# keio-bioinformatics/stem_kernel

Measured on AMD Instinct MI355X. Metric: sequence-pairs/sec (Gram entries/s) at L=200 nt, higher is better.
Workload: dtype f64

## Files before the change

stem_kernel_amd/csrc/kernels/dag_stem.hip:

```cpp
#include <hip/hip_runtime.h>

#include <algorithm>

#include "device_set.h"
#include "launch.h"

namespace sk {

__global__ void sk_prep_kernel(DevSet s, DevParamNodes pn, const double* __restrict__ gpow,
                               double gap2) {
  const int e = blockIdx.x * blockDim.x + threadIdx.x;
  if (e >= s.n_examples) return;
  const int nl = s.ex_nl[e];
  const int nb = s.ex_node_base[e], eb = s.ex_edge_base[e];
  for (int k = 0; k < nl; ++k) {
    const uint32_t a = s.nd_a[nb + k];
    const int e0 = a & 0xffff, ne = (a >> 16) & 0xff;
    const double v_s = gap2 * (double)s.nd_w[nb + k];
    double L = 0.0, SL = 0.0;
    if (ne == 0) {
      L += 1.0 * v_s * gpow[s.nd_c[nb + k]];
    } else {
      for (int t = 0; t < ne; ++t) {
        const uint32_t ed = s.ed[eb + e0 + t].x;
        const double gp = gpow[ed >> 16];
        const double Lc = pn.nd_L[nb + (ed & 0xffff)];
        L += Lc * v_s * gp;
        SL += gp * Lc;
      }
    }
    pn.nd_L[nb + k] = L;
    pn.nd_SL[nb + k] = SL;
  }
  for (int r = 0; r < nl; ++r) pn.xr_SL[nb + r] = pn.nd_SL[nb + s.xr_node[nb + r]];
  {
    int k = s.ex_xch_base[e];
    for (int r = 0; r < nl; ++r) {
      const int ne = s.xrow[nb + r].a & 0xff;
      for (int t = 0; t < ne; ++t, ++k) pn.xr_chw[k] = gpow[s.xr_ch[k] >> 16];
    }
  }
  if (s.n_gam > 0) {
    const int gb = s.ex_xg_base[e], nlg = s.ex_nlxg[e];
    int k = s.ex_xgch_base[e];
    int pk = s.n_phi > 0 ? s.ex_phk_base[e] : 0;
    for (int r = 0; r < nlg; ++r) {
      const double SLr = pn.nd_SL[nb + s.xg_node[gb + r]];
      pn.xg_SL[gb + r] = SLr;
      const XRow xr = s.xgrow[gb + r];
      const int ne = xr.a & 0xff;
      for (int t = 0; t < ne; ++t, ++k) {
        const uint32_t c = s.xg_ch[k];
        const double wc = gpow[c >> 16] * gpow[s.xg_clg[k]] * (double)s.xg_cpf[k];
        double w;
        switch (s.xg_cty[k]) {
          case 0: w = gpow[c >> 16]; break;
          case 1: w = wc; break;
          case 2: w = (double)xr.bp0 * wc; break;
          case 3: w = (double)xr.bp0 * SLr; break;
          default: w = gap2 * (double)xr.w * wc; break;
        }
        pn.xg_chw[k] = w;
        if (s.xg_cty[k] == 2) pn.phk_w[pk++] = xr.P * w;
      }
    }
    double* h = pn.gam_h + (int64_t)e * s.n_gam;
    for (int g = 0; g < s.n_gam; ++g) h[g] = 0.0;
    for (int i = s.ex_gr_base[e]; i < s.ex_gr_base[e + 1]; ++i) {
      const uint32_t inf = s.gr_info[i];
      h[inf & 0xffff] += s.gr_P[i] * (gpow[inf >> 16] * (double)s.gr_pf[i]);
    }
    if (s.n_phi > 0)
      for (int i = s.ex_gra_base[e]; i < s.ex_gra_base[e + 1]; ++i) {
        const uint32_t r = s.gra_row[i];
        h[s.gra_gidx[i]] += s.xgrow[r].P * ((double)s.xgrow[r].bp0 * pn.xg_SL[r]);
      }
  }
}

typedef __attribute__((address_space(3))) double lds_f64;
typedef __attribute__((address_space(3))) float lds_f32;
typedef __attribute__((address_space(3))) uint32_t lds_u32;
typedef __attribute__((address_space(3))) int32_t lds_i32;

struct YView {
  const uint4* __restrict__ nrg;
  const lds_u32* sc;
  const lds_f64* ew;
  const lds_f32* ewf;
  const lds_f64* gp;
  double gap2;
  const lds_u32* ed2;
  const uint32_t* __restrict__ ed2g;
  const lds_i32* lfirst;
  const lds_i32* ycs;
  int lmax;
  int nl, nch;
  float nseqs;
  int nb, bb;
};

#if defined(__HIP_DEVICE_COMPILE__)
template <typename T>
using cst_ptr = const __attribute__((address_space(4))) T*;
#else
template <typename T>
using cst_ptr = const T*;
#endif

__device__ __forceinline__ void wave_sync() {
  __builtin_amdgcn_fence(__ATOMIC_RELEASE, "wavefront");
  __builtin_amdgcn_wave_barrier();
  __builtin_amdgcn_fence(__ATOMIC_ACQUIRE, "wavefront");
}

#define SCHED_FENCE() __builtin_amdgcn_sched_barrier(0)
#ifndef SK_W20
#define SK_W20 8
#endif
#ifndef SK_W16
#define SK_W16 8
#endif
#ifndef SK_NPF12
#define SK_NPF12 2
#endif
#ifndef SK_NPF20
#define SK_NPF20 2
#endif
#ifndef SK_NPF16
#define SK_NPF16 1
#endif
#ifndef SK_NPF17
#define SK_NPF17 0
#endif
#ifndef SK_PW
#define SK_PW 3
#endif
#ifndef SK_SEGSUM
#define SK_SEGSUM 1
#endif
#ifndef SK_SEGSUM_MAXK
#define SK_SEGSUM_MAXK 20
#endif
#ifndef SK_MU
#define SK_MU 3
#endif
#ifndef SK_NODEW_MIN
#define SK_NODEW_MIN 20
#endif
#ifndef SK_M16
#define SK_M16 1
#endif
#ifndef SK_K17
#define SK_K17 1
#endif
template <int MAXK>
constexpr bool m16_wide() {
  return (MAXK == 16 || MAXK == 17) && SK_M16 != 0;
}
template <int MAXK>
constexpr bool node_weights() {
  return MAXK >= SK_NODEW_MIN || m16_wide<MAXK>();
}
#ifndef SK_NODEF_MIN
#define SK_NODEF_MIN 24
#endif
template <int MAXK>
constexpr bool node_weights_f32() {
  return node_weights<MAXK>() && MAXK >= SK_NODEF_MIN;
}
#ifndef SK_PW2_MIN
#define SK_PW2_MIN 24
#endif
template <int MAXK>
#ifndef SK_PW17
#define SK_PW17 2
#endif
constexpr int pass_width() {
  return MAXK == 17 ? SK_PW17 : (MAXK >= SK_PW2_MIN || m16_wide<MAXK>()) ? 2 : SK_PW;
}
static inline bool m16_wide_of(int maxk) { return (maxk == 16 || maxk == 17) && SK_M16 != 0; }
static inline int pass_width_of(int maxk) {
  return maxk == 17 ? SK_PW17 : (maxk >= SK_PW2_MIN || m16_wide_of(maxk)) ? 2 : SK_PW;
}
static inline bool node_weights_of(int maxk) { return maxk >= SK_NODEW_MIN || m16_wide_of(maxk); }
#ifndef SK_EDG_MIN
#define SK_EDG_MIN 64
#endif
template <int MAXK>
constexpr bool edges_global() {
  return MAXK >= SK_EDG_MIN;
}

#ifdef SK_STAMPS
#define STAMP(i)                                                  \
  do {                                                            \
    __builtin_amdgcn_sched_barrier(0);                            \
    const unsigned long long _t = __builtin_amdgcn_s_memtime();   \
    tacc[i] += _t - tlast;                                        \
    tlast = _t;                                                   \
    __builtin_amdgcn_sched_barrier(0);                            \
  } while (0)
#else
#define STAMP(i) do {} while (0)
#endif

__device__ __forceinline__ double match_node_score(const lds_f64* co, const DevSet& s, int xbb,
                                                int xb0, int xnb, const DevSet& ys, const YView& Y,
                                                int yb0, int ynb, double xwg, double ywg,
                                                double x_nbp, double y_nbp, double x_nseq) {
  double v = 0.0;
  for (int a = 0; a < xnb; ++a) {
    const double cx = (double)s.bpf_p[xbb + xb0 + a];
    const uint32_t ca = s.bpf_code[xbb + xb0 + a] * 16u;
    for (int b = 0; b < ynb; ++b) {
      const double cy = (double)ys.bpf_p[Y.bb + yb0 + b];
      v += co[ca + ys.bpf_code[Y.bb + yb0 + b]] * cx * cy;
    }
  }
  v += ywg * x_nbp / x_nseq;
  v += xwg * y_nbp / (double)Y.nseqs;
  return v;
}

__device__ __forceinline__ __amdgpu_buffer_rsrc_t row_rsrc(const double* base, int nly) {
  const uint64_t a = (uint64_t)base;
  const uint32_t lo = __builtin_amdgcn_readfirstlane((uint32_t)a);
  const uint32_t hi = __builtin_amdgcn_readfirstlane((uint32_t)(a >> 32));
  return __builtin_amdgcn_make_buffer_rsrc((void*)(((uint64_t)hi << 32) | lo), (short)0,
                                           __builtin_amdgcn_readfirstlane(nly * 8), 0x00020000);
}

#ifndef SK_ROW_LD_POL
#define SK_ROW_LD_POL 0
#endif
#ifndef SK_ROW_ST_POL
#define SK_ROW_ST_POL 0
#endif
typedef unsigned int u32x2 __attribute__((__vector_size__(2 * sizeof(unsigned int))));

__device__ __forceinline__ double row_ld(__amdgpu_buffer_rsrc_t r, int lane, int k) {
  return __builtin_bit_cast(double, __builtin_amdgcn_raw_buffer_load_b64(r, lane * 8, k * 512, SK_ROW_LD_POL));
}

#ifndef SK_HALF_A
#define SK_HALF_A 64
#endif
#ifndef SK_HALF_D
#define SK_HALF_D 64
#endif
#ifndef SK_M16_HALFA
#define SK_M16_HALFA 1
#endif
#ifndef SK_M16_HALFD
#define SK_M16_HALFD 1
#endif
template <int MAXK>
__device__ __forceinline__ void add_rows2(double (&S)[MAXK], __amdgpu_buffer_rsrc_t r0,
                                          __amdgpu_buffer_rsrc_t r1, double eg0, double eg1,
                                          int lane) {
  constexpr int H = (MAXK > SK_HALF_A || (m16_wide<MAXK>() && SK_M16_HALFA)) ? (MAXK + 1) / 2 : MAXK;
#pragma unroll
  for (int h0 = 0; h0 < MAXK; h0 += H) {
    double a[H], b[H];
#pragma unroll
    for (int k = 0; k < H; ++k) {
      a[k] = h0 + k < MAXK ? row_ld(r0, lane, h0 + k) : 0.0;
      b[k] = h0 + k < MAXK ? row_ld(r1, lane, h0 + k) : 0.0;
    }
    SCHED_FENCE();
#pragma unroll
    for (int k = 0; k < H; ++k)
      if (h0 + k < MAXK) S[h0 + k] += eg0 * a[k] + eg1 * b[k];
  }
}

template <bool NW, bool NWF>
__device__ __forceinline__ void iy_sweep(const YView& Y, lds_f64* R, int c0, int lane) {
  const lds_u32* rp = Y.sc + c0 * 64 + lane;
  const lds_f64* wp = Y.ew + (NW ? 0 : c0 * 64 + lane);
  auto nweight = [&](uint32_t rec) __attribute__((always_inline)) -> double {
    const uint32_t pa = (rec >> 11) & 0x7ff;
    return (NWF ? Y.gap2 * (double)Y.ewf[pa] : Y.ew[pa]) * Y.gp[rec >> 22];
  };
  struct Ck {
    uint32_t rec;
    double w, rv;
  };
  Ck A, B, C;
  A.rec = rp[0];
  B.rec = rp[64];
  A.w = NW ? nweight(A.rec) : wp[0];
  B.w = 0.0;
  C.rec = 0u;
  C.w = C.rv = B.rv = 0.0;
  A.rv = R[A.rec & 0x7ff];
  int c = c0;
  const int nch = Y.nch;
  auto step = [&](Ck& X, Ck& Yc, Ck& Z) __attribute__((always_inline)) -> bool {
    Z.rec = rp[128];
    Yc.w = NW ? nweight(Yc.rec) : wp[64];
    __hip_atomic_fetch_add(&R[(X.rec >> 11) & 0x7ff], X.rv * X.w, __ATOMIC_RELAXED,
                           __HIP_MEMORY_SCOPE_WAVEFRONT);
    Yc.rv = R[Yc.rec & 0x7ff];
    rp += 64;
    wp += 64;
    return ++c < nch;
  };
  for (;;) {
    if (!step(A, B, C)) break;
    if (!step(B, C, A)) break;
    if (!step(C, A, B)) break;
  }
  wave_sync();
}

__device__ __forceinline__ const double* child_row(uint32_t c, const double* slab, const double* gamtab,
                                                   const double* phitab, int stride) {
  const double* base = (c & 0x8000u) ? gamtab : (c & 0x4000u) ? phitab : slab;
  return base + (size_t)(c & 0x3fffu) * stride;
}

template <int MAXK>
__device__ double stem_pair(const StemLaunch& P, const YView& Y, lds_f64* R, lds_f64* hb,
                            const lds_f64* co, const lds_f64* gp, double* __restrict__ slab, int x,
                            int lane, bool gam, const double* __restrict__ gamtab,
                            const lds_f64* kap, const double* __restrict__ phitab,
                            const double* __restrict__ phikap) {
  constexpr int stride = 64 * MAXK;
  constexpr int PW = pass_width<MAXK>();
  const DevSet& s = P.xset;
  const DevSet& ys = P.yset;
  const double* __restrict__ yPg = ys.yn_P + Y.nb;
  const int NLy = Y.nl;
  if (s.ex_nl[x] == 0 || NLy == 0) return 0.0;
  const int xnb = s.ex_node_base[x], xbb = s.ex_bpf_base[x];
  const int xgb = gam ? s.ex_xg_base[x] : 0;
  const int nlx = gam ? s.ex_nlxg[x] : s.ex_nl[x];
  int chp = gam ? s.ex_xgch_base[x] : s.ex_xch_base[x];
  const double x_nseq = (double)s.ex_nseqs[x];
  const double gap2 = P.gap2;
  const int band = (int)P.band;
  const XRow* __restrict__ xrows = gam ? s.xgrow + xgb : s.xrow + xnb;
  const double* __restrict__ xsl = gam ? P.pn.xg_SL + xgb : P.pn.xr_SL + xnb;
  const uint32_t* __restrict__ xch = gam ? s.xg_ch : s.xr_ch;
  const double* __restrict__ xchw = gam ? P.pn.xg_chw : P.pn.xr_chw;
  double kacc = 0.0;
  if (gam) {
    const double* __restrict__ h = P.pn.gam_h + (int64_t)x * s.n_gam;
    for (int g = lane; g < s.n_gam; g += 64) kacc += h[g] * kap[g];
    if (P.phi_on)
      for (int j = s.ex_phk_base[x] + lane; j < s.ex_phk_base[x + 1]; j += 64)
        kacc += P.pn.phk_w[j] * phikap[s.phk_idx[j]];
  }
  if (nlx == 0) {
    for (int off = 32; off > 0; off >>= 1) kacc += __shfl_xor(kacc, off, 64);
    return kacc;
  }
#ifdef SK_STAMPS
  unsigned long long tacc[8] = {0, 0, 0, 0, 0, 0, 0, 0};
  unsigned long long cnt[4] = {0, 0, 0, 0};
  unsigned long long tlast = __builtin_amdgcn_s_memtime();
#endif

  const cst_ptr<XRow> xrows_c = (cst_ptr<XRow>)xrows;
  const cst_ptr<double> xsl_c = (cst_ptr<double>)xsl;
  const cst_ptr<uint32_t> xch_c = (cst_ptr<uint32_t>)xch;
  const cst_ptr<double> xchw_c = (cst_ptr<double>)xchw;
  XRow nx = xrows_c[0];
  double nSL = xsl_c[0];
  uint32_t nch[4];
  double ncw[4];
#pragma unroll
  for (int j = 0; j < 4; ++j) {
    nch[j] = xch_c[chp + j];
    ncw[j] = xchw_c[chp + j];
  }

  double S[MAXK];
#pragma unroll
  for (int k = 0; k < MAXK; ++k) S[k] = 0.0;
  uint32_t done = 0;

  for (int r = 0; r < nlx; ++r) {
    const uint32_t xa = nx.a, xb = nx.b, xc = nx.c;
    const double xwg = gap2 * (double)nx.w;
    const double x_nbp = (double)nx.nbp;
    const double xP = nx.P, xSL = nSL, xpf = (double)nx.bp0;
    uint32_t ch[4];
    double cw[4];
#pragma unroll
    for (int j = 0; j < 4; ++j) {
      ch[j] = nch[j];
      cw[j] = ncw[j];
    }
    const int xne = xa & 0xff, xnbf = (xa >> 8) & 0xff;
    const int chp_r = chp;
    chp += xne;
    const int xlen = xb & 0xffff;
    const uint32_t pslot = xb >> 16;
    const int xb0 = xc & 0xffff;
    const bool xloop = xne == 0;
    const double xeg0 = gp[xa >> 16];
    const bool x_one = xnbf == 1 && x_nbp == 0.0;
    const uint32_t xcode = ((xc >> 16) & 0xffu) * 16u;
    const bool combo = (xc >> 31) != 0u;
    int qa = 0, qb = NLy;
    if (band > 0) {
      qa = Y.lfirst[min(max(xlen - band, 0), Y.lmax + 1)];
      qb = Y.lfirst[min(max(xlen + band + 1, 0), Y.lmax + 1)];
    }
    qa = __builtin_amdgcn_readfirstlane(qa);
    qb = __builtin_amdgcn_readfirstlane(qb);
    uint4 nd_first[PW];
    double Pq_first[PW];
#pragma unroll
    for (int j = 0; j < PW; ++j) {
      nd_first[j] = make_uint4(0u, 0u, 0u, 0u);
      Pq_first[j] = 0.0;
    }
    if (qa < qb) {
#pragma unroll
      for (int j = 0; j < PW; ++j) {
        const int qf = min(max(qb - 64 * PW, qa) + 64 * j + lane, qb - 1);
        nd_first[j] = Y.nrg[qf];
        Pq_first[j] = yPg[qf];
      }
    }
    STAMP(0);

    SCHED_FENCE();
    if (r + 1 < nlx) {
      nx = xrows_c[r + 1];
      nSL = xsl_c[r + 1];
#pragma unroll
      for (int j = 0; j < 4; ++j) {
        nch[j] = xch_c[chp + j];
        ncw[j] = xchw_c[chp + j];
      }
    }
    SCHED_FENCE();

    {
      uint32_t c[4] = {0u, 0u, 0u, 0u};
      double w[4] = {0.0, 0.0, 0.0, 0.0};
      int na = 0;
#pragma unroll
      for (int j = 0; j < 4; ++j) {
        const bool take = j < xne && !(done >> j & 1u);
        c[0] = (take && na == 0) ? ch[j] : c[0];
        c[1] = (take && na == 1) ? ch[j] : c[1];
        c[2] = (take && na == 2) ? ch[j] : c[2];
        c[3] = (take && na == 3) ? ch[j] : c[3];
        w[0] = (take && na == 0) ? cw[j] : w[0];
        w[1] = (take && na == 1) ? cw[j] : w[1];
        w[2] = (take && na == 2) ? cw[j] : w[2];
        w[3] = (take && na == 3) ? cw[j] : w[3];
        na += take ? 1 : 0;
      }
      for (int h = 0; h < 4; h += 2) {
        if (na > h) {
          const bool two = na > h + 1;
          const uint32_t c0 = c[h], c1 = two ? c[h + 1] : c[h];
          const double eg0 = w[h], eg1 = two ? w[h + 1] : 0.0;
          add_rows2<MAXK>(S, row_rsrc(child_row(c0, slab, gamtab, phitab, stride), NLy),
                          row_rsrc(child_row(c1, slab, gamtab, phitab, stride), NLy), eg0, eg1, lane);
        }
      }
    }
#ifdef SK_STAMPS
    {
      int nl_ = 0;
      for (int j = 0; j < 4; ++j) nl_ += (j < xne && !(done >> j & 1u)) ? 1 : 0;
      cnt[0] += nl_ + (xne > 4 ? xne - 4 : 0);
    }
#endif
    for (int t = 4; t < xne; t += 2) {
      const uint32_t c0 = xch[chp_r + t];
      const bool two = t + 1 < xne;
      const uint32_t c1 = two ? xch[chp_r + t + 1] : c0;
      const double eg0 = xchw[chp_r + t], eg1 = two ? xchw[chp_r + t + 1] : 0.0;
      add_rows2<MAXK>(S, row_rsrc(child_row(c0, slab, gamtab, phitab, stride), NLy),
                      row_rsrc(child_row(c1, slab, gamtab, phitab, stride), NLy), eg0, eg1, lane);
    }
    STAMP(1);

    if (!combo) {
#pragma unroll
      for (int k = 0; k < MAXK; ++k) R[lane + 64 * k] = lane + 64 * k < qb ? S[k] : 0.0;
    }
    double rowk = 0.0;
    STAMP(2);
#ifdef SK_STAMPS
    cnt[3] += qb > qa ? qb - qa : 0;
#endif
    if (!combo && qa < qb) {
      constexpr int NW = 64 * PW;
      int top = qb - 1, q0 = max(top - NW + 1, qa);
      uint4 nd_n[PW];
      double Pq_n[PW];
#pragma unroll
      for (int j = 0; j < PW; ++j) {
        nd_n[j] = nd_first[j];
        Pq_n[j] = Pq_first[j];
      }
      for (;;) {
        uint4 nd[PW];
        double Pq[PW];
#pragma unroll
        for (int j = 0; j < PW; ++j) {
          nd[j] = nd_n[j];
          Pq[j] = Pq_n[j];
        }
        const int ntop = top - NW, nq0 = max(ntop - NW + 1, qa);
        if (ntop >= qa) {
#pragma unroll
          for (int j = 0; j < PW; ++j) {
            nd_n[j] = Y.nrg[min(nq0 + 64 * j + lane, ntop)];
            Pq_n[j] = yPg[min(nq0 + 64 * j + lane, ntop)];
          }
        }
        double co_v[PW], gl_v[PW];
#pragma unroll
        for (int j = 0; j < PW; ++j) {
          co_v[j] = co[xcode + ((nd[j].y >> 16) & 0xf)];
          gl_v[j] = gp[nd[j].y & 0xffff];
        }
        double Hq[PW];
#pragma unroll
        for (int j = 0; j < PW; ++j) Hq[j] = 0.0;
        if (!xloop) {
          const int ea = __builtin_amdgcn_readfirstlane(nd[0].x & 0xffff);
          const int jt = (top - q0) >> 6;
          uint32_t ndt = nd[0].x;
#pragma unroll
          for (int j = 1; j < PW; ++j) ndt = jt == j ? nd[j].x : ndt;
          const uint32_t at = __builtin_amdgcn_readlane(ndt, (top - q0) & 63);
          const int eb = (int)((at & 0xffff) + ((at >> 16) & 0xff));
          constexpr bool EG = edges_global<MAXK>();
          uint32_t en[SK_MU];
          if constexpr (EG) {
#pragma unroll
            for (int u = 0; u < SK_MU; ++u) en[u] = Y.ed2g[min(ea + 64 * u + lane, eb - 1)];
          }
          for (int f0 = ea; f0 < eb; f0 += 64 * SK_MU) {
            uint32_t e[SK_MU];
            if constexpr (EG) {
#pragma unroll
              for (int u = 0; u < SK_MU; ++u) {
                e[u] = en[u];
                en[u] = Y.ed2g[min(f0 + 64 * (SK_MU + u) + lane, eb - 1)];
              }
            } else {
#pragma unroll
              for (int u = 0; u < SK_MU; ++u) e[u] = Y.ed2[min(f0 + 64 * u + lane, eb - 1)];
            }
            double g[SK_MU], rv[SK_MU];
#pragma unroll
            for (int u = 0; u < SK_MU; ++u) {
              g[u] = gp[e[u] >> 22];
              rv[u] = R[e[u] & 0x7ff];
            }
#pragma unroll
            for (int u = 0; u < SK_MU; ++u) {
              const bool ok = f0 + 64 * u + lane < eb;
              const double w = g[u] * rv[u] * (ok ? 1.0 : 0.0);
              const int h = ok ? (int)((e[u] >> 11) & 0x7ff) - q0 : lane;
              if constexpr (SK_SEGSUM && MAXK <= SK_SEGSUM_MAXK) {
                const int key = ok ? h : -1 - lane;
                const int ql = lane & 3;
                double sw = w;
                {
                  const int ks = __builtin_amdgcn_mov_dpp(key, 0x90, 0xf, 0xf, false);
                  const double ws = __hiloint2double(
                      __builtin_amdgcn_mov_dpp(__double2hiint(sw), 0x90, 0xf, 0xf, false),
                      __builtin_amdgcn_mov_dpp(__double2loint(sw), 0x90, 0xf, 0xf, false));
                  sw += (ql >= 1 && ks == key) ? ws : 0.0;
                }
                {
                  const int ks = __builtin_amdgcn_mov_dpp(key, 0x40, 0xf, 0xf, false);
                  const double ws = __hiloint2double(
                      __builtin_amdgcn_mov_dpp(__double2hiint(sw), 0x40, 0xf, 0xf, false),
                      __builtin_amdgcn_mov_dpp(__double2loint(sw), 0x40, 0xf, 0xf, false));
                  sw += (ql >= 2 && ks == key) ? ws : 0.0;
                }
                const int kn = __builtin_amdgcn_mov_dpp(key, 0xF9, 0xf, 0xf, false);
                if (ok && (ql == 3 || kn != key))
                  __hip_atomic_fetch_add(&hb[h], sw, __ATOMIC_RELAXED, __HIP_MEMORY_SCOPE_WAVEFRONT);
              } else {
                __hip_atomic_fetch_add(&hb[h], w, __ATOMIC_RELAXED, __HIP_MEMORY_SCOPE_WAVEFRONT);
              }
            }
          }
#pragma unroll
          for (int j = 0; j < PW; ++j) {
            Hq[j] = hb[64 * j + lane];
            hb[64 * j + lane] = 0.0;
          }
        }
#pragma unroll
        for (int j = 0; j < PW; ++j) {
          const int q = q0 + 64 * j + lane;
          const bool on = q <= top;
          const uint32_t nda = nd[j].x, ndc = nd[j].y;
          double H = Hq[j];
          if (((nda >> 16) & 0xff) == 0)
            H = (xloop ? xeg0 : xSL) * gl_v[j];
          double vs;
          if (x_one && (ndc >> 24) != 0u) {
            vs = co_v[j] * xpf * (double)__uint_as_float(nd[j].w);
          } else {
            const int qq = on ? q : top;
            vs = H != 0.0 ? match_node_score(co, s, xbb, xb0, xnbf, ys, Y, ys.yn_b[Y.nb + qq] >> 16,
                                             nda >> 24, xwg, gap2 * (double)__uint_as_float(nd[j].z),
                                             x_nbp, (double)ys.yn_nbp[Y.nb + qq], x_nseq)
                          : 0.0;
          }
          const double M = vs * H;
          if (on) {
            R[q] = M;
            rowk += M * Pq[j];
          }
        }
#ifdef SK_STAMPS
        cnt[2] += 1;
#endif
        if (ntop < qa) break;
        top = ntop;
        q0 = nq0;
      }
    }
    STAMP(3);
#pragma unroll
    for (int k = 0; k < MAXK; ++k) {
      const int q = lane + 64 * k;
      if (!combo && 64 * k < qa && q < qa) R[q] = 0.0;
    }
    kacc += xP * rowk;
    wave_sync();
    STAMP(4);

    constexpr int NPF = MAXK == 17 ? SK_NPF17
                        : (MAXK == 16 && (SK_NPF16 == 0 || SK_M16 == 2)) ? 0
                        : ((MAXK <= 12 && SK_NPF12 == 2) || (MAXK == 16 && SK_NPF16 == 2) ||
                           (MAXK == 20 && SK_W20 == 8 && SK_NPF20 == 2)) ? 2 : 1;
    uint32_t nxt_done = 0;
    double egd = 0.0, egt0 = 0.0, egt1 = 0.0;
    double T0[MAXK], T1[MAXK];
#pragma unroll
    for (int k = 0; k < MAXK; ++k) T0[k] = T1[k] = 0.0;
    if (r + 1 < nlx) {
      const int nne = nx.a & 0xff;
      uint32_t pf0 = 0, pf1 = 0;
      int npf = 0;
#pragma unroll
      for (int j = 0; j < 4; ++j) {
        if (j < nne) {
          const uint32_t c = nch[j];
          const double g = ncw[j];
          if ((c & 0xffff) == pslot) {
            egd += g;
            nxt_done |= 1u << j;
          } else if (npf < NPF) {
            if (npf == 0) {
              pf0 = c;
              egt0 = g;
            } else {
              pf1 = c;
              egt1 = g;
            }
            ++npf;
            nxt_done |= 1u << j;
          }
        }
      }
      if (NPF >= 1 && npf >= 1) {
        const __amdgpu_buffer_rsrc_t r0 = row_rsrc(child_row(pf0, slab, gamtab, phitab, stride), NLy);
#pragma unroll
        for (int k = 0; k < MAXK; ++k) T0[k] = row_ld(r0, lane, k);
      }
      if (NPF >= 2 && npf >= 2) {
        const __amdgpu_buffer_rsrc_t r1 = row_rsrc(child_row(pf1, slab, gamtab, phitab, stride), NLy);
#pragma unroll
        for (int k = 0; k < MAXK; ++k) T1[k] = row_ld(r1, lane, k);
      }
    }

    int c0 = 0;
    if (band > 0) c0 = Y.ycs[min(max(xlen - band, 0), Y.lmax + 1)];
    c0 = __builtin_amdgcn_readfirstlane(c0);
#ifdef SK_STAMPS
    cnt[1] += Y.nch - c0;
#endif
    if (!combo && c0 < Y.nch && pslot != 0xffffu) {
      iy_sweep<node_weights<MAXK>(), node_weights_f32<MAXK>()>(Y, R, c0, lane);
      wave_sync();
    }
    STAMP(5);

    constexpr int HD = (MAXK > SK_HALF_D || (m16_wide<MAXK>() && SK_M16_HALFD)) ? (MAXK + 1) / 2 : MAXK;
    if (pslot == 0xffffu) {
#pragma unroll
      for (int k = 0; k < MAXK; ++k) S[k] = egt0 * T0[k] + (NPF >= 2 ? egt1 * T1[k] : 0.0);
    } else if (pslot == 0xfffeu) {
      const double cw = combo ? 1.0 : xwg;
#pragma unroll
      for (int h0 = 0; h0 < MAXK; h0 += HD) {
        double g1[HD];
#pragma unroll
        for (int k = 0; k < HD; ++k) g1[k] = combo ? 0.0 : R[lane + 64 * (h0 + k)];
        SCHED_FENCE();
#pragma unroll
        for (int k = 0; k < HD; ++k)
          S[h0 + k] = egd * (g1[k] + cw * S[h0 + k]) + egt0 * T0[h0 + k] + (NPF >= 2 ? egt1 * T1[h0 + k] : 0.0);
      }
    } else {
#ifdef SK_FULL_STORE
      double* __restrict__ orow = slab + (size_t)pslot * stride + lane;
#else
      const __amdgpu_buffer_rsrc_t orsrc = row_rsrc(slab + (size_t)pslot * stride, NLy);
#endif
      const double cw = combo ? 1.0 : xwg;
#pragma unroll
      for (int h0 = 0; h0 < MAXK; h0 += HD) {
        double g1[HD];
#pragma unroll
        for (int k = 0; k < HD; ++k) g1[k] = combo ? 0.0 : R[lane + 64 * (h0 + k)];
        SCHED_FENCE();
#pragma unroll
        for (int k = 0; k < HD; ++k) {
          const double o = g1[k] + cw * S[h0 + k];
#ifndef SK_XNOSTORE
#ifdef SK_FULL_STORE
          orow[64 * (h0 + k)] = o;
#else
          __builtin_amdgcn_raw_buffer_store_b64(__builtin_bit_cast(u32x2, o), orsrc, lane * 8,
                                                (h0 + k) * 512, SK_ROW_ST_POL);
#endif
#endif
          S[h0 + k] = egd * o + egt0 * T0[h0 + k] + (NPF >= 2 ? egt1 * T1[h0 + k] : 0.0);
        }
      }
    }
    done = nxt_done;
    wave_sync();
    STAMP(6);
  }
#ifdef SK_STAMPS
  if (lane == 0 && P.stamps) {
    for (int i = 0; i < 8; ++i) atomicAdd(&P.stamps[i], tacc[i]);
    atomicAdd(&P.stamps[8], (unsigned long long)nlx);
    atomicAdd(&P.stamps[9], 1ull);
    for (int i = 0; i < 4; ++i) atomicAdd(&P.stamps[10 + i], cnt[i]);
  }
#endif
  for (int off = 32; off > 0; off >>= 1) kacc += __shfl_xor(kacc, off, 64);
  return kacc;
}

template <int MAXK>
struct StemWaves {
  static constexpr int value = MAXK <= 12 ? 12 : MAXK <= 17 ? (SK_M16 ? 12 : SK_W16) : MAXK <= 20 ? SK_W20 : 8;
};

struct StemLds {
  lds_f64* co;
  lds_f64* gp;
  lds_f64* Rall;
  lds_f64* hball;
  lds_f64* yew;
  lds_u32* ysc;
  lds_u32* yed2;
  lds_i32* ylf;
  lds_i32* ycs;
  lds_i32* ctl;
  lds_f64* kap;
};

template <int MAXK>
__device__ __forceinline__ StemLds stem_lds_carve(const StemLaunch& P, int nwaves) {
  extern __shared__ __attribute__((aligned(16))) unsigned char smem[];
  const int maxnl = P.lds_max_nl;
  constexpr int PW = pass_width<MAXK>();
  constexpr bool NW = node_weights<MAXK>();
  StemLds L;
  L.co = (lds_f64*)(smem);
  L.gp = L.co + 256;
  L.Rall = L.gp + P.n_gpow_pad;
  L.hball = L.Rall + (size_t)nwaves * maxnl;
  L.yew = L.hball + (size_t)nwaves * 64 * PW;
  L.ysc = (lds_u32*)(L.yew + (node_weights_f32<MAXK>() ? (size_t)maxnl / 2
                              : NW ? (size_t)maxnl : (size_t)P.lds_max_nch * 64));
  L.yed2 = L.ysc + (size_t)P.lds_max_nch * 64;
  L.ylf = (lds_i32*)(L.yed2 + (edges_global<MAXK>() ? 0 : P.lds_max_edges));
  L.ycs = L.ylf + P.lds_max_len_pad;
  L.ctl = L.ycs + P.lds_max_len_pad;
  L.kap = (lds_f64*)(L.ctl + 4);
  return L;
}

template <int MAXK>
__device__ __forceinline__ void stage_y(const StemLaunch& P, const StemLds& L, int y, YView& Y) {
  const DevSet& s = P.yset;
  constexpr bool NW = node_weights<MAXK>();
  const int maxnl = P.lds_max_nl;
  const double gap2 = P.gap2;
  lds_f64* gp = L.gp;
  lds_f64* yew = L.yew;
  lds_u32* ysc = L.ysc;
  lds_u32* yed2 = L.yed2;
  lds_i32* ylf = L.ylf;
  lds_i32* ycs = L.ycs;
  {
    Y.nl = s.ex_nl[y];
    Y.nch = s.ex_nch[y];
    Y.nseqs = s.ex_nseqs[y];
    const int nb = s.ex_node_base[y], eb = s.ex_edge_base[y], bb = s.ex_bpf_base[y];
    Y.lmax = Y.nl ? (int)(s.yn_b[nb + Y.nl - 1] & 0xffff) : 0;
    {
      const int ne = s.ex_edge_base[y + 1] - eb;
      const int sb = s.ex_ysc_base[y] * 64, nrec = Y.nch * 64;
      const int nfree = max(maxnl - Y.nl, 1);
      for (int k = threadIdx.x; k < nrec + 128; k += blockDim.x) {
        uint32_t r = k < nrec ? s.ysc[sb + k] : 0u;
        const uint32_t ch = r & 0x7ff, pa = (r >> 11) & 0x7ff;
        const uint32_t zs = (uint32_t)(maxnl - 1 - (k & 63) % nfree);
        if (k >= nrec || ch == pa) r = zs | (zs << 11);
        ysc[k] = r;
        if (!NW) yew[k] = (k >= nrec || ch == pa) ? 0.0 : gap2 * (double)s.yn_w[nb + pa] * gp[r >> 22];
      }
      if (node_weights_f32<MAXK>())
        for (int q = threadIdx.x; q < maxnl; q += blockDim.x) ((lds_f32*)yew)[q] = q < Y.nl ? s.yn_w[nb + q] : 0.0f;
      else if (NW)
        for (int q = threadIdx.x; q < maxnl; q += blockDim.x) yew[q] = q < Y.nl ? gap2 * (double)s.yn_w[nb + q] : 0.0;
      if (!edges_global<MAXK>())
        for (int k = threadIdx.x; k < ne; k += blockDim.x) yed2[k] = s.ye2[eb + k];
      const int cb = s.ex_ycs_base[y];
      for (int v = threadIdx.x; v <= Y.lmax + 1; v += blockDim.x) ycs[v] = s.ycs[cb + v];
    }
    Y.nrg = s.yrec + nb;
    Y.sc = ysc; Y.ew = yew; Y.ed2 = yed2; Y.lfirst = ylf; Y.ycs = ycs; Y.gp = gp;
    Y.ewf = (const lds_f32*)yew; Y.gap2 = gap2;
    Y.ed2g = s.ye2 + eb;
    Y.nb = nb; Y.bb = bb;
    __syncthreads();
    for (int v = threadIdx.x; v <= Y.lmax + 1; v += blockDim.x) {
      int lo = 0, hi = Y.nl;
      while (lo < hi) {
        const int mid = (lo + hi) >> 1;
        if ((int)(s.yn_b[nb + mid] & 0xffff) < v) lo = mid + 1; else hi = mid;
      }
      ylf[v] = lo;
    }
    __syncthreads();
  }
}

template <int MAXK, typename KapPtr>
__device__ __forceinline__ void gamma_rows(const StemLaunch& P, const YView& Y, lds_f64* R, const lds_f64* co,
                                           const lds_f64* gp, double* gamtab, KapPtr kap, int wave_u,
                                           int nwaves, int lane) {
  const DevSet& s = P.yset;
  const DevSet& xset = P.xset;
  const int band = (int)P.band;
  const int nb = Y.nb, bb = Y.bb;
  for (int g = wave_u; g < xset.n_gam; g += nwaves) {
    const uint32_t key = xset.gam_key[g];
    const int gcode = (int)(key >> 16) * 16, glen = (int)(key & 0xffff);
    double kp = 0.0;
    for (int k = 0; k < MAXK; ++k) {
      const int q = lane + 64 * k;
      double M = 0.0;
      if (q < Y.nl) {
        const uint4 nd = Y.nrg[q];
        const int ylen = (int)(s.yn_b[nb + q] & 0xffff);
        if (((nd.x >> 16) & 0xff) == 0 && (band == 0 || abs(glen - ylen) <= band)) {
          double vs;
          if ((nd.y >> 24) != 0u) {
            vs = co[gcode + ((nd.y >> 16) & 0xf)] * (double)__uint_as_float(nd.w);
          } else {
            vs = 0.0;
            const int yb0 = (int)(s.yn_b[nb + q] >> 16), ynb = (int)(nd.x >> 24);
            for (int b = 0; b < ynb; ++b)
              vs += co[gcode + s.bpf_code[bb + yb0 + b]] * (double)s.bpf_p[bb + yb0 + b];
          }
          M = vs * gp[nd.y & 0xffff];
          kp += M * s.yn_P[nb + q];
        }
      }
      R[q] = M;
    }
    for (int off = 32; off > 0; off >>= 1) kp += __shfl_xor(kp, off, 64);
    if (lane == 0) kap[g] = kp;
    wave_sync();
    int c0 = 0;
    if (band > 0) c0 = Y.ycs[min(max(glen - band, 0), Y.lmax + 1)];
    c0 = __builtin_amdgcn_readfirstlane(c0);
    if (c0 < Y.nch) iy_sweep<node_weights<MAXK>(), node_weights_f32<MAXK>()>(Y, R, c0, lane);
    double* grow = gamtab + (size_t)g * (64 * MAXK);
    for (int k = 0; k < MAXK; ++k)
      if (lane + 64 * k < Y.nl) grow[lane + 64 * k] = R[lane + 64 * k];
    wave_sync();
  }
}

template <int MAXK>
__device__ __forceinline__ void phi_rows(const StemLaunch& P, const YView& Y, lds_f64* R, const lds_f64* co,
                                         const lds_f64* gp, const double* gamtab, double* phitab,
                                         double* phikap, const int32_t* __restrict__ keys, int pb, int pe,
                                         int wave_u, int nwaves, int lane) {
  const DevSet& s = P.yset;
  const DevSet& xset = P.xset;
  const int band = (int)P.band;
  const int nb = Y.nb, bb = Y.bb;
  const int share = (pe - pb + nwaves - 1) / nwaves;
  const int t0 = pb + wave_u * share, t1 = min(pe, t0 + share);
  int gcur = -1;
  double Hr[MAXK];
#pragma unroll
  for (int k = 0; k < MAXK; ++k) Hr[k] = 0.0;
  for (int t = t0; t < t1; ++t) {
    const int idx = keys ? __builtin_amdgcn_readfirstlane(keys[t]) : t;
    const int g = __builtin_amdgcn_readfirstlane((int)xset.phi_g[idx]);
    if (g != gcur) {
      gcur = g;
      const double* __restrict__ grow = gamtab + (size_t)g * (64 * MAXK);
#pragma unroll
      for (int k = 0; k < MAXK; ++k) R[lane + 64 * k] = grow[lane + 64 * k];
      wave_sync();
      for (int k = 0; k < MAXK; ++k) {
        const int q = lane + 64 * k;
        double H = 0.0;
        if (q < Y.nl) {
          const uint32_t na = Y.nrg[q].x;
          const int ne = (int)((na >> 16) & 0xff), e0 = (int)(na & 0xffff);
          for (int e = 0; e < ne; ++e) {
            const uint32_t rec = edges_global<MAXK>() ? Y.ed2g[e0 + e] : Y.ed2[e0 + e];
            H += gp[rec >> 22] * R[rec & 0x7ff];
          }
        }
        Hr[k] = H;
      }
      wave_sync();
    }
    const uint32_t al = xset.phi_al[idx];
    const int acode = (int)(al >> 16) * 16, alen = (int)(al & 0xffff);
    double kp = 0.0;
#pragma unroll
    for (int k = 0; k < MAXK; ++k) {
      const int q = lane + 64 * k;
      double M = 0.0;
      if (q < Y.nl) {
        const uint4 nd = Y.nrg[q];
        const int ylen = (int)(s.yn_b[nb + q] & 0xffff);
        if (Hr[k] != 0.0 && (band == 0 || abs(alen - ylen) <= band)) {
          double vs;
          if ((nd.y >> 24) != 0u) {
            vs = co[acode + ((nd.y >> 16) & 0xf)] * (double)__uint_as_float(nd.w);
          } else {
            vs = 0.0;
            const int yb0 = (int)(s.yn_b[nb + q] >> 16), ynb = (int)(nd.x >> 24);
            for (int b = 0; b < ynb; ++b)
              vs += co[acode + s.bpf_code[bb + yb0 + b]] * (double)s.bpf_p[bb + yb0 + b];
          }
          M = vs * Hr[k];
          kp += M * s.yn_P[nb + q];
        }
      }
      R[q] = M;
    }
    for (int off = 32; off > 0; off >>= 1) kp += __shfl_xor(kp, off, 64);
    if (lane == 0) phikap[idx] = kp;
    wave_sync();
    int c0 = 0;
    if (band > 0) c0 = Y.ycs[min(max(alen - band, 0), Y.lmax + 1)];
    c0 = __builtin_amdgcn_readfirstlane(c0);
    if (c0 < Y.nch) iy_sweep<node_weights<MAXK>(), node_weights_f32<MAXK>()>(Y, R, c0, lane);
    double* prow = phitab + (size_t)idx * (64 * MAXK);
#pragma unroll
    for (int k = 0; k < MAXK; ++k)
      if (lane + 64 * k < Y.nl) prow[lane + 64 * k] = R[lane + 64 * k];
    wave_sync();
  }
}

template <int MAXK>
__global__ void __launch_bounds__(64 * StemWaves<MAXK>::value) sk_gamma_table_kernel(StemLaunch P) {
  const int lane = threadIdx.x & 63, wave = threadIdx.x >> 6;
  const int nwaves = blockDim.x >> 6;
  const int slot = blockIdx.x;
  if (slot >= P.n_slots) return;
  const StemLds L = stem_lds_carve<MAXK>(P, nwaves);
  for (int k = threadIdx.x; k < 256; k += blockDim.x) L.co[k] = P.co_subst[k];
  for (int k = threadIdx.x; k < P.n_gpow; k += blockDim.x) L.gp[k] = P.gpow[k];
  lds_f64* R = L.Rall + (size_t)wave * P.lds_max_nl;
  const int wave_u = __builtin_amdgcn_readfirstlane(wave);
  __syncthreads();
  YView Y;
  stage_y<MAXK>(P, L, P.slot_y[slot], Y);
  double* gamtab = P.gam + (size_t)slot * P.gam_doubles;
  gamma_rows<MAXK>(P, Y, R, L.co, L.gp, gamtab, P.kap_y + (size_t)slot * P.xset.n_gam, wave_u, nwaves, lane);
  if (P.phi_shared) {
    __syncthreads();
    double* phitab = P.phi + (size_t)slot * P.phi_doubles;
    phi_rows<MAXK>(P, Y, R, L.co, L.gp, gamtab, phitab, phitab + (size_t)P.xset.n_phi * (64 * MAXK), nullptr, 0,
                   P.xset.n_phi, wave_u, nwaves, lane);
  }
}

template <int MAXK>
__global__ void __launch_bounds__(64 * StemWaves<MAXK>::value) sk_dag_stem_kernel(StemLaunch P) {
  const DevSet& s = P.yset;
  const int lane = threadIdx.x & 63, wave = threadIdx.x >> 6;
  const int nwaves = blockDim.x >> 6;
  const int maxnl = P.lds_max_nl;
  constexpr int PW = pass_width<MAXK>();

  const StemLds L = stem_lds_carve<MAXK>(P, nwaves);
  lds_f64* co = L.co;
  lds_f64* gp = L.gp;
  lds_i32* ctl = L.ctl;
  lds_f64* kap = L.kap;

  for (int k = threadIdx.x; k < 256; k += blockDim.x) co[k] = P.co_subst[k];
  for (int k = threadIdx.x; k < P.n_gpow; k += blockDim.x) gp[k] = P.gpow[k];

  lds_f64* R = L.Rall + (size_t)wave * maxnl;
  lds_f64* hb = L.hball + (size_t)wave * 64 * PW;
  for (int j = 0; j < PW; ++j) hb[64 * j + lane] = 0.0;
  double* slab = P.scratch + (size_t)(blockIdx.x * nwaves + wave) * P.slab_doubles;
  const int wave_u = __builtin_amdgcn_readfirstlane(wave);
  if (threadIdx.x == 0) ctl[2] = 0;
  for (;;) {
    __syncthreads();
    if (threadIdx.x == 0) {
      int got = -1, qk = ctl[2];
      while (qk < kStemQueues) {
        const int q = (blockIdx.x + qk) % kStemQueues;
        const int i = P.queue_off[q] + atomicAdd(P.item_counter + q, 1);
        if (i < P.queue_off[q + 1]) {
          got = i;
          break;
        }
        ++qk;
      }
      ctl[0] = got;
      ctl[2] = qk;
    }
    __syncthreads();
    const int it = __builtin_amdgcn_readfirstlane(ctl[0]);
    if (it < 0) break;
    const int4 item = P.items[it];
    const int y = item.x;
    YView Y;
    stage_y<MAXK>(P, L, y, Y);

    const bool gam = P.gam_on && s.ex_gapless[y];
    double* gamtab = nullptr;
    const int tslot = __builtin_amdgcn_readfirstlane(P.phi_shared ? item.w : (int)blockIdx.x);
    double* phitab = P.phi + (int64_t)tslot * P.phi_doubles;
    double* phikap = P.phi_on ? phitab + (size_t)P.xset.n_phi * (64 * MAXK) : nullptr;
    if (gam) {
      const DevSet& xset = P.xset;
      if (P.gam_shared) {
        gamtab = P.gam + (size_t)item.w * P.gam_doubles;
        const double* __restrict__ ky = P.kap_y + (size_t)item.w * xset.n_gam;
        for (int g = threadIdx.x; g < xset.n_gam; g += blockDim.x) kap[g] = ky[g];
      } else {
        gamtab = P.gam + (size_t)blockIdx.x * P.gam_doubles;
        gamma_rows<MAXK>(P, Y, R, co, gp, gamtab, kap, wave_u, nwaves, lane);
      }
      __syncthreads();

      if (P.phi_on && !P.phi_shared) {
        phi_rows<MAXK>(P, Y, R, co, gp, gamtab, phitab, phikap, P.item_phi, P.item_phi_off[it],
                       P.item_phi_off[it + 1], wave_u, nwaves, lane);
        __syncthreads();
      }
    }

    if (threadIdx.x == 0) ctl[1] = nwaves;
    __syncthreads();
    for (int t = wave_u; t < item.z;) {
      const int x = P.xs[item.y + t];
      const double k = stem_pair<MAXK>(P, Y, R, hb, co, gp, slab, x, lane, gam, gamtab, kap, phitab, phikap);
      if (lane == 0) P.out[P.oidx[item.y + t]] = k;
      int nt = 0;
      if (lane == 0) nt = atomicAdd(reinterpret_cast<int*>(const_cast<int32_t*>((const int32_t*)ctl)) + 1, 1);
      t = __builtin_amdgcn_readlane(nt, 0);
    }
  }
}

hipError_t launch_prep(const DevSet& s, const DevParamNodes& pn, const double* gpow, double gap2,
                       hipStream_t st) {
  const int bs = 64;
  const int grid = (s.n_examples + bs - 1) / bs;
  if (grid == 0) return hipSuccess;
  hipLaunchKernelGGL(sk_prep_kernel, dim3(grid), dim3(bs), 0, st, s, pn, gpow, gap2);
  return hipGetLastError();
}

size_t stem_lds_bytes(const StemLaunch& P, int nwaves) {
  size_t b = 0;
  b += 256 * 8;
  b += (size_t)P.n_gpow_pad * 8;
  b += (size_t)nwaves * P.lds_max_nl * 8;
  b += (size_t)nwaves * 64 * pass_width_of(stem_maxk(P.lds_max_nl)) * 8;
  const int maxk = stem_maxk(P.lds_max_nl);
  if (node_weights_of(maxk))
    b += (size_t)P.lds_max_nch * 64 * 4 + (size_t)P.lds_max_nl * (maxk >= SK_NODEF_MIN ? 4 : 8);
  else
    b += (size_t)P.lds_max_nch * 64 * 12;
  if (stem_maxk(P.lds_max_nl) < SK_EDG_MIN) b += (size_t)P.lds_max_edges * 4;
  b += (size_t)P.lds_max_len_pad * 4 * 2 + 16;
  if (P.gam_on) b += (size_t)P.xset.n_gam * 8;
  return b;
}

#define SK_STEM_CLASSES(X) X(4) X(8) X(12) X(16) X(17) X(20) X(24) X(28) X(32)

static const void* stem_kernel_ptr(int maxk) {
  switch (maxk) {
#define SK_CASE(K) \
  case K: return reinterpret_cast<const void*>(sk_dag_stem_kernel<K>);
    SK_STEM_CLASSES(SK_CASE)
#undef SK_CASE
    default: return nullptr;
  }
}

int stem_maxk(int max_nl) {
  const int s = (std::max(max_nl, 1) + 63) / 64;
  if (SK_K17 && s == 17) return 17;
  const int k = (s + 3) & ~3;
  return k <= 32 ? k : -1;
}

hipError_t launch_stem(const StemLaunch& P, int grid, int nwaves, hipStream_t st) {
  const size_t lds = stem_lds_bytes(P, nwaves);
  const int maxk = stem_maxk(P.lds_max_nl);
  const void* fn = stem_kernel_ptr(maxk);
  if (!fn) return hipErrorInvalidValue;
  hipError_t e = hipFuncSetAttribute(fn, hipFuncAttributeMaxDynamicSharedMemorySize, (int)lds);
  if (e != hipSuccess) return e;
  switch (maxk) {
#define SK_CASE(K)                                                                          \
  case K:                                                                                  \
    hipLaunchKernelGGL(sk_dag_stem_kernel<K>, dim3(grid), dim3(64 * nwaves), lds, st, P); \
    break;
    SK_STEM_CLASSES(SK_CASE)
#undef SK_CASE
    default: return hipErrorInvalidValue;
  }
  return hipGetLastError();
}

hipError_t launch_gamma_tables(const StemLaunch& P, int nwaves, hipStream_t st) {
  if (!P.gam_shared || P.n_slots <= 0) return hipSuccess;
  const size_t lds = stem_lds_bytes(P, nwaves);
  const int maxk = stem_maxk(P.lds_max_nl);
  switch (maxk) {
#define SK_CASE(K)                                                                                  \
  case K: {                                                                                        \
    hipError_t e = hipFuncSetAttribute(reinterpret_cast<const void*>(sk_gamma_table_kernel<K>),    \
                                       hipFuncAttributeMaxDynamicSharedMemorySize, (int)lds);      \
    if (e != hipSuccess) return e;                                                                 \
    hipLaunchKernelGGL(sk_gamma_table_kernel<K>, dim3(P.n_slots), dim3(64 * nwaves), lds, st, P); \
    break;                                                                                         \
  }
    SK_STEM_CLASSES(SK_CASE)
#undef SK_CASE
    default: return hipErrorInvalidValue;
  }
  return hipGetLastError();
}

hipError_t stem_kernel_attr(int max_nl, int* max_dyn_lds, int* vgprs, int* max_waves) {
  hipFuncAttributes attr;
  const int maxk = stem_maxk(max_nl);
  if (maxk < 0) return hipErrorInvalidValue;
  hipError_t e = hipFuncGetAttributes(&attr, stem_kernel_ptr(maxk));
  if (e != hipSuccess) return e;
  *max_dyn_lds = 163840 - (int)attr.sharedSizeBytes;
  *vgprs = attr.numRegs;
  *max_waves = std::max(1, attr.maxThreadsPerBlock / 64);
  return hipSuccess;
}

}
```

Measured before the change: 227,500.

## Software-pipeline child row accumulation across pairs with rotating load windows

Replaces the per-pair add_rows2 calls with a unified loop over all child pairs that splits each row into units and keeps the loads of the next units in flight while the current ones are accumulated, including across pair boundaries. The extra children beyond four are prefetched cooperatively, one per lane, and broadcast with readlane instead of being loaded serially from memory. The aim is to hide buffer-load latency between consecutive row reads. The cost is more live registers for the double-buffered windows and more complex control flow, which could lower occupancy.

```diff
diff --git a/stem_kernel_amd/csrc/kernels/dag_stem.hip b/stem_kernel_amd/csrc/kernels/dag_stem.hip
--- a/stem_kernel_amd/csrc/kernels/dag_stem.hip
+++ b/stem_kernel_amd/csrc/kernels/dag_stem.hip
@@ -243,36 +243,67 @@
   return __builtin_bit_cast(double, __builtin_amdgcn_raw_buffer_load_b64(r, lane * 8, k * 512, SK_ROW_LD_POL));
 }
 
-#ifndef SK_HALF_A
-#define SK_HALF_A 64
+#ifndef SK_A_UNITS_M16
+#define SK_A_UNITS_M16 4
+#endif
+#ifndef SK_A_UNITS
+#define SK_A_UNITS 2
 #endif
 #ifndef SK_HALF_D
 #define SK_HALF_D 64
 #endif
-#ifndef SK_M16_HALFA
-#define SK_M16_HALFA 1
-#endif
 #ifndef SK_M16_HALFD
 #define SK_M16_HALFD 1
 #endif
 template <int MAXK>
-__device__ __forceinline__ void add_rows2(double (&S)[MAXK], __amdgpu_buffer_rsrc_t r0,
-                                          __amdgpu_buffer_rsrc_t r1, double eg0, double eg1,
-                                          int lane) {
-  constexpr int H = (MAXK > SK_HALF_A || (m16_wide<MAXK>() && SK_M16_HALFA)) ? (MAXK + 1) / 2 : MAXK;
-#pragma unroll
-  for (int h0 = 0; h0 < MAXK; h0 += H) {
-    double a[H], b[H];
-#pragma unroll
-    for (int k = 0; k < H; ++k) {
-      a[k] = h0 + k < MAXK ? row_ld(r0, lane, h0 + k) : 0.0;
-      b[k] = h0 + k < MAXK ? row_ld(r1, lane, h0 + k) : 0.0;
-    }
-    SCHED_FENCE();
-#pragma unroll
-    for (int k = 0; k < H; ++k)
-      if (h0 + k < MAXK) S[h0 + k] += eg0 * a[k] + eg1 * b[k];
-  }
+struct AWindow {
+  static constexpr int NU = m16_wide<MAXK>() ? SK_A_UNITS_M16 : SK_A_UNITS;
+  static_assert(NU >= 2 && NU % 2 == 0 && NU <= MAXK, "two groups take the units in turn");
+  static constexpr int lo(int u) { return u * (MAXK / NU) + (u < MAXK % NU ? u : MAXK % NU); }
+  static constexpr int C0 = lo(1) - lo(0), C1 = lo(2) - lo(1);
+  double a0[C0], b0[C0], a1[C1], b1[C1];
+
+  template <int U>
+  __device__ __forceinline__ void issue(__amdgpu_buffer_rsrc_t r0, __amdgpu_buffer_rsrc_t r1, int lane) {
+    constexpr int L = lo(U), N = lo(U + 1) - L;
+#pragma unroll
+    for (int k = 0; k < N; ++k) {
+      if constexpr (U % 2 == 0) {
+        a0[k] = row_ld(r0, lane, L + k);
+        b0[k] = row_ld(r1, lane, L + k);
+      } else {
+        a1[k] = row_ld(r0, lane, L + k);
+        b1[k] = row_ld(r1, lane, L + k);
+      }
+    }
+  }
+  template <int U>
+  __device__ __forceinline__ void add(double (&S)[MAXK], double eg0, double eg1) const {
+    constexpr int L = lo(U), N = lo(U + 1) - L;
+#pragma unroll
+    for (int k = 0; k < N; ++k) {
+      if constexpr (U % 2 == 0)
+        S[L + k] += eg0 * a0[k] + eg1 * b0[k];
+      else
+        S[L + k] += eg0 * a1[k] + eg1 * b1[k];
+    }
+  }
+  template <int U, int E>
+  __device__ __forceinline__ void steps(double (&S)[MAXK], double eg0, double eg1, __amdgpu_buffer_rsrc_t r0,
+                                        __amdgpu_buffer_rsrc_t r1, int lane) {
+    if constexpr (U < E) {
+      add<U>(S, eg0, eg1);
+      SCHED_FENCE();
+      issue<(U + 2) % NU>(r0, r1, lane);
+      SCHED_FENCE();
+      steps<U + 1, E>(S, eg0, eg1, r0, r1, lane);
+    }
+  }
+};
+
+__device__ __forceinline__ double readlane_f64(double v, int l) {
+  return __hiloint2double(__builtin_amdgcn_readlane(__double2hiint(v), l),
+                          __builtin_amdgcn_readlane(__double2loint(v), l));
 }
 
 template <bool NW, bool NWF>
@@ -412,6 +443,13 @@
     }
     qa = __builtin_amdgcn_readfirstlane(qa);
     qb = __builtin_amdgcn_readfirstlane(qb);
+    uint32_t rc = 0u;
+    double rw = 0.0;
+    if (xne > 4) {
+      const int j = chp_r + 4 + min(lane, xne - 5);
+      rc = xch[j];
+      rw = xchw[j];
+    }
     uint4 nd_first[PW];
     double Pq_first[PW];
 #pragma unroll
@@ -458,30 +496,63 @@
         w[3] = (take && na == 3) ? cw[j] : w[3];
         na += take ? 1 : 0;
       }
-      for (int h = 0; h < 4; h += 2) {
-        if (na > h) {
-          const bool two = na > h + 1;
-          const uint32_t c0 = c[h], c1 = two ? c[h + 1] : c[h];
-          const double eg0 = w[h], eg1 = two ? w[h + 1] : 0.0;
-          add_rows2<MAXK>(S, row_rsrc(child_row(c0, slab, gamtab, phitab, stride), NLy),
-                          row_rsrc(child_row(c1, slab, gamtab, phitab, stride), NLy), eg0, eg1, lane);
+#ifdef SK_STAMPS
+      cnt[0] += na + (xne > 4 ? xne - 4 : 0);
+#endif
+      int npf = (na + 1) >> 1;
+      for (int tb = 4;;) {
+        const int nrec = min(max(xne - tb, 0), 64);
+        const int np = npf + ((nrec + 1) >> 1);
+        auto pair_at = [&](int p, bool lanes, __amdgpu_buffer_rsrc_t& q0, __amdgpu_buffer_rsrc_t& q1,
+                           double& g0, double& g1) __attribute__((always_inline)) {
+          const bool first = p < npf;
+          const int t = 2 * (p - npf);
+          const uint32_t ra = lanes ? __builtin_amdgcn_readlane(rc, t & 63) : 0u;
+          const uint32_t rb = lanes ? __builtin_amdgcn_readlane(rc, (t + 1) & 63) : 0u;
+          const double wa = lanes ? readlane_f64(rw, t & 63) : 0.0;
+          const double wb = lanes ? readlane_f64(rw, (t + 1) & 63) : 0.0;
+          const bool ha = first || t < nrec;
+          const bool hb = first ? 2 * p + 1 < na : t + 1 < nrec;
+          const uint32_t ca = first ? (p == 0 ? c[0] : c[2]) : ra;
+          const uint32_t cb = first ? (p == 0 ? c[1] : c[3]) : rb;
+          g0 = !ha ? 0.0 : first ? (p == 0 ? w[0] : w[2]) : wa;
+          g1 = !hb ? 0.0 : first ? (p == 0 ? w[1] : w[3]) : wb;
+          q0 = row_rsrc(child_row(ha ? ca : 0u, slab, gamtab, phitab, stride), ha ? NLy : 0);
+          q1 = row_rsrc(child_row(hb ? cb : 0u, slab, gamtab, phitab, stride), hb ? NLy : 0);
+        };
+        if (np > 0) {
+          AWindow<MAXK> W;
+          __amdgpu_buffer_rsrc_t r0, r1;
+          double eg0, eg1;
+          if (npf > 0)
+            pair_at(0, false, r0, r1, eg0, eg1);
+          else
+            pair_at(0, true, r0, r1, eg0, eg1);
+          W.template issue<0>(r0, r1, lane);
+          SCHED_FENCE();
+          W.template issue<1>(r0, r1, lane);
+          SCHED_FENCE();
+          constexpr int NU = AWindow<MAXK>::NU;
+          for (int p = 1; p < np; ++p) {
+            double ng0, ng1;
+            W.template steps<0, NU - 2>(S, eg0, eg1, r0, r1, lane);
+            pair_at(p, true, r0, r1, ng0, ng1);
+            W.template steps<NU - 2, NU>(S, eg0, eg1, r0, r1, lane);
+            eg0 = ng0;
+            eg1 = ng1;
+          }
+          W.template steps<0, NU - 2>(S, eg0, eg1, r0, r1, lane);
+          W.template add<NU - 2>(S, eg0, eg1);
+          W.template add<NU - 1>(S, eg0, eg1);
         }
-      }
-    }
-#ifdef SK_STAMPS
-    {
-      int nl_ = 0;
-      for (int j = 0; j < 4; ++j) nl_ += (j < xne && !(done >> j & 1u)) ? 1 : 0;
-      cnt[0] += nl_ + (xne > 4 ? xne - 4 : 0);
-    }
-#endif
-    for (int t = 4; t < xne; t += 2) {
-      const uint32_t c0 = xch[chp_r + t];
-      const bool two = t + 1 < xne;
-      const uint32_t c1 = two ? xch[chp_r + t + 1] : c0;
-      const double eg0 = xchw[chp_r + t], eg1 = two ? xchw[chp_r + t + 1] : 0.0;
-      add_rows2<MAXK>(S, row_rsrc(child_row(c0, slab, gamtab, phitab, stride), NLy),
-                      row_rsrc(child_row(c1, slab, gamtab, phitab, stride), NLy), eg0, eg1, lane);
+        tb += 64;
+        if (tb >= xne) break;
+        const int j = chp_r + tb + min(lane, xne - tb - 1);
+        rc = xch[j];
+        rw = xchw[j];
+        npf = 0;
+        na = 0;
+      }
     }
     STAMP(1);
 
```

Result: no change. 229,100, median of 6 (+0.7%).
